# p2004dr/visual-slam

Hardware: AMD Instinct MI355X
Metric: frames/sec (extract+match+pose) at 640×480, 2000 ORB, 1/2/4/8 MI355X (higher is better)
Workload: dtype u8

## Files before the change

visual-slam_amd/csrc/orb_kernels.hip:

```cpp
#include <cstring>

#include "common.h"
#include "select_replay.h"

__constant__ __attribute__((aligned(16))) int8_t c_pattern[256 * 4] = {
#include "orb_pattern.inc"
};

#define WAVE 64

__device__ __forceinline__ int reflect101(int p, int len) {
    if (len == 1) return 0;
    while (p < 0 || p >= len) p = p < 0 ? -p : 2 * len - 2 - p;
    return p;
}

__device__ __forceinline__ void xcd_map(uint32_t lin, uint32_t per, uint32_t inv_per, uint32_t batch, int& frame, int& item) {
    const uint32_t b8 = batch & ~7u, cut = per * b8;
    const bool head = lin < cut;
    const uint32_t n = head ? lin >> 3 : lin - cut;
    const uint32_t q = inv_per ? __umulhi(n, inv_per) : n;
    item = (int)(n - q * per);
    frame = (int)(head ? (lin & 7u) + 8u * q : b8 + q);
}

__device__ __forceinline__ const uint8_t* level_ptr(const Plan& P, int L, const uint8_t* gray, const uint8_t* pyr,
                                                    int frame) {
    return L == 0 ? gray + (size_t)frame * P.w * P.h : pyr + (size_t)frame * P.pyr_stride + P.lv[L].off;
}

__global__ void k_gray(const uint8_t* __restrict__ bgr, uint8_t* __restrict__ gray, size_t npx) {
    size_t i = (size_t)blockIdx.x * blockDim.x + threadIdx.x;
    if (i >= npx) return;
    int b = bgr[3 * i], g = bgr[3 * i + 1], r = bgr[3 * i + 2];
    gray[i] = (uint8_t)((b * 3735 + g * 19235 + r * 9798 + (1 << 14)) >> 15);
}

int orb_launch_gray(mo_ctx* c, const uint8_t* d_bgr, int w, int h, int batch, uint8_t* d_gray) {
    size_t npx = (size_t)w * h * batch;
    hipLaunchKernelGGL(k_gray, dim3((unsigned)((npx + 255) / 256)), dim3(256), 0, c->stream, d_bgr, d_gray, npx);
    HIPCHK(c, hipGetLastError());
    return MO_OK;
}

__global__ __launch_bounds__(256) void k_ingest(const uint8_t* __restrict__ src, uint8_t* __restrict__ gray, int npx, int ch, int* flags_clear) {
    const int i = (blockIdx.x * 256 + threadIdx.x) * 16;
    if (blockIdx.x == 0 && threadIdx.x == 0 && flags_clear) { flags_clear[0] = 0; flags_clear[1] = 0; flags_clear[2] = 0; flags_clear[3] = 0; }
    if (i >= npx) return;
    if (i + 16 <= npx) {
        if (ch == 1) {
            *(uint4*)(gray + i) = *(const uint4*)(src + i);
        } else {
            const uint4* s4 = (const uint4*)(src + (size_t)3 * i);
            const uint4 a = s4[0], b = s4[1], c = s4[2];
            const uint32_t wsrc[12] = {a.x, a.y, a.z, a.w, b.x, b.y, b.z, b.w, c.x, c.y, c.z, c.w};
            uint32_t o[4];
#pragma unroll
            for (int q = 0; q < 4; q++) {
                uint32_t v = 0;
#pragma unroll
                for (int k = 0; k < 4; k++) {
                    const int byte = 3 * (4 * q + k);
                    const uint32_t bb = (wsrc[byte >> 2] >> (8 * (byte & 3))) & 255u, gg = (wsrc[(byte + 1) >> 2] >> (8 * ((byte + 1) & 3))) & 255u,
                                   rr = (wsrc[(byte + 2) >> 2] >> (8 * ((byte + 2) & 3))) & 255u;
                    v |= ((bb * 3735u + gg * 19235u + rr * 9798u + (1u << 14)) >> 15) << (8 * k);
                }
                o[q] = v;
            }
            *(uint4*)(gray + i) = make_uint4(o[0], o[1], o[2], o[3]);
        }
        return;
    }
    for (int j = i; j < npx; j++) {
        if (ch == 1) gray[j] = src[j];
        else gray[j] = (uint8_t)(((int)src[3 * (size_t)j] * 3735 + (int)src[3 * (size_t)j + 1] * 19235 + (int)src[3 * (size_t)j + 2] * 9798 + (1 << 14)) >> 15);
    }
}

int orb_launch_ingest(mo_ctx* c, const uint8_t* src_mapped, int w, int h, int ch, uint8_t* d_gray, int* flags_clear) {
    const int npx = w * h;
    hipLaunchKernelGGL(k_ingest, dim3((unsigned)((npx + 4095) / 4096)), dim3(256), 0, c->stream, src_mapped, d_gray, npx, ch, flags_clear);
    HIPCHK(c, hipGetLastError());
    return MO_OK;
}

typedef unsigned short u16x2 __attribute__((ext_vector_type(2)));
__device__ __forceinline__ uint32_t udot2(uint32_t a, uint32_t b, uint32_t c) {
    return __builtin_amdgcn_udot2(__builtin_bit_cast(u16x2, a), __builtin_bit_cast(u16x2, b), c, false);
}

#define RS_TW 64
#define RS_TH 64
#define RS_SRC_ROWS 136
#define RS_SRC_PITCH 144

__global__ __launch_bounds__(256) void k_resize(const uint8_t* __restrict__ src, size_t src_fstride, int spitch, int sw, int sh,
                                                uint8_t* __restrict__ dst, size_t dst_fstride, int dpitch, int dw, int dh,
                                                const int* __restrict__ xofs, const int* __restrict__ xc1,
                                                const int* __restrict__ yofs, const int* __restrict__ yc1,
                                                uint32_t inv_per, uint32_t inv_gx, int org) {
    __shared__ __attribute__((aligned(16))) uint8_t s_src[RS_SRC_ROWS * RS_SRC_PITCH];
    __shared__ int s_xo[RS_TW], s_xc[RS_TW], s_yo[RS_TH], s_yc[RS_TH];
    const int tid = threadIdx.x;
    int bx = blockIdx.x, by = blockIdx.y, bz = blockIdx.z;
    {
        int rem;
        xcd_map(bx + gridDim.x * (by + gridDim.y * bz), gridDim.x * gridDim.y, inv_per, gridDim.z, bz, rem);
        by = (int)(inv_gx ? __umulhi((uint32_t)rem, inv_gx) : (uint32_t)rem);
        bx = rem - by * (int)gridDim.x;
    }
    const int tx0 = org + bx * RS_TW, ty0 = org + by * RS_TH;
    const uint8_t* s = src + (size_t)bz * src_fstride;
    const int sx0 = xofs[tx0], sx1 = min(xofs[min(tx0 + RS_TW - 1, dw - 1)] + 1, sw - 1);
    const int sy0 = yofs[ty0], sy1 = min(yofs[min(ty0 + RS_TH - 1, dh - 1)] + 1, sh - 1);
    const int sxa = sx0 & ~3;
    const int ncols = sx1 - sxa + 1, nrows = sy1 - sy0 + 1;
    if (ncols > RS_SRC_PITCH || nrows > RS_SRC_ROWS) return;
    if (tid < RS_TW) {
        int x = min(tx0 + tid, dw - 1);
        s_xo[tid] = xofs[x];
        s_xc[tid] = xc1[x];
    } else if (tid < RS_TW + RS_TH) {
        int y = min(ty0 + tid - RS_TW, dh - 1);
        s_yo[tid - RS_TW] = yofs[y];
        s_yc[tid - RS_TW] = yc1[y];
    }
    if ((spitch & 3) == 0 && (((size_t)s) & 3) == 0) {
        const int ndw = (ncols + 3) >> 2;
        const uint32_t inv = 0x100000u / (uint32_t)ndw + 1u;
        const uint8_t* s0 = s + (size_t)sy0 * spitch + sxa;
        for (int i = tid; i < nrows * ndw; i += 256) {
            const uint32_t r = ((uint32_t)i * inv) >> 20, c4 = (uint32_t)i - r * (uint32_t)ndw;
            ((uint32_t*)(s_src + r * RS_SRC_PITCH))[c4] = *(const uint32_t*)(s0 + r * (uint32_t)spitch + 4u * c4);
        }
    } else {
        for (int i = tid; i < nrows * ncols; i += 256) {
            int r = i / ncols, cc = i - r * ncols;
            s_src[r * RS_SRC_PITCH + cc] = s[(size_t)(sy0 + r) * spitch + sxa + cc];
        }
    }
    __syncthreads();
    const int c0 = (tid & 15) * 4, x = tx0 + c0;
    if (x >= dw) return;
    int ox[4], ox1[4];
    uint32_t mx1[4];
#pragma unroll
    for (int k = 0; k < 4; k++) {
        ox[k] = s_xo[c0 + k] - sxa;
        ox1[k] = min(s_xo[c0 + k] + 1, sw - 1) - sxa;
        mx1[k] = s_xc[c0 + k];
    }
#pragma unroll
    for (int half = 0; half < RS_TH / 16; half++) {
        const int ry = (tid >> 4) + 16 * half, y = ty0 + ry;
        if (y >= dh) break;
        const int oy = s_yo[ry] - sy0, oy1 = min(s_yo[ry] + 1, sh - 1) - sy0;
        const uint32_t my1 = s_yc[ry], my0 = 256 - my1;
        const uint8_t* r0 = s_src + oy * RS_SRC_PITCH;
        const uint8_t* r1 = s_src + oy1 * RS_SRC_PITCH;
        uint32_t packed = 0;
#pragma unroll
        for (int k = 0; k < 4; k++) {
            const uint32_t mx0 = 256 - mx1[k];
            uint32_t h0 = mx0 * r0[ox[k]] + mx1[k] * r0[ox1[k]];
            uint32_t h1 = mx0 * r1[ox[k]] + mx1[k] * r1[ox1[k]];
            uint32_t v = my0 * h0 + my1 * h1;
            packed |= ((v + 32768u) >> 16) << (8 * k);
        }
        *(uint32_t*)(dst + (size_t)bz * dst_fstride + (size_t)y * dpitch + x) = packed;
    }
}


#define RS2_ROWS 136
#define RS2_UNR 5
__global__ __launch_bounds__(256) void k_resize2(const uint8_t* __restrict__ src, size_t src_fstride, int spitch, int sw, int sh,
                                                 uint8_t* __restrict__ dst, size_t dst_fstride, int dpitch, int dw, int dh,
                                                 const uint32_t* __restrict__ xpk, const uint32_t* __restrict__ ypk,
                                                 uint32_t inv_per, uint32_t inv_gx, int org) {
    __shared__ __attribute__((aligned(16))) uint2 s_h[RS2_ROWS][16];
    const int tid = threadIdx.x;
    int bx = blockIdx.x, by = blockIdx.y, bz = blockIdx.z;
    {
        int rem;
        xcd_map(bx + gridDim.x * (by + gridDim.y * bz), gridDim.x * gridDim.y, inv_per, gridDim.z, bz, rem);
        by = (int)(inv_gx ? __umulhi((uint32_t)rem, inv_gx) : (uint32_t)rem);
        bx = rem - by * (int)gridDim.x;
    }
    const int tx0 = org + bx * RS_TW, ty0 = org + by * RS_TH;
    const uint32_t ey0 = ypk[ty0], ey1 = ypk[min(ty0 + RS_TH - 1, dh - 1)];
    const int sy0 = (int)(ey0 & 0x7FFFu), sy1 = (int)(ey1 & 0x7FFFu) + (int)((ey1 >> 15) & 1u);
    const int nrows = sy1 - sy0 + 1;
    if (nrows > RS2_ROWS) return;
    const int cg = tid & 15, rr = tid >> 4;
    const uint4 xe = *(const uint4*)(xpk + tx0 + 4 * cg);
    uint32_t ye[RS_TH / 16];
#pragma unroll
    for (int half = 0; half < RS_TH / 16; half++) ye[half] = ypk[ty0 + rr + 16 * half];
    const uint32_t xk[4] = {xe.x, xe.y, xe.z, xe.w};
    const int ox0 = (int)(xk[0] & 0x7FFFu), ab = ox0 & ~3;
    const uint32_t sh8 = (uint32_t)(ox0 & 3);
    uint32_t sel[4], coef[4];
#pragma unroll
    for (int k = 0; k < 4; k++) {
        const uint32_t a = (xk[k] & 0x7FFFu) - (uint32_t)ox0, b = a + ((xk[k] >> 15) & 1u), c1 = xk[k] >> 16;
        sel[k] = a | (b << 16) | 0x0C000C00u;
        coef[k] = (256u - c1) | (c1 << 16);
    }
    const int o1 = min(ab + 4, spitch - 4), o2 = min(ab + 8, spitch - 4);
    const uint8_t* s0 = src + (size_t)bz * src_fstride + (size_t)sy0 * spitch;
    for (int r0 = rr; r0 < nrows; r0 += 16 * RS2_UNR) {
        uint32_t w[RS2_UNR][3];
#pragma unroll
        for (int i = 0; i < RS2_UNR; i++) {
            const uint8_t* row = s0 + (uint32_t)(min(r0 + 16 * i, nrows - 1) * spitch);
            w[i][0] = *(const uint32_t*)(row + ab); w[i][1] = *(const uint32_t*)(row + o1); w[i][2] = *(const uint32_t*)(row + o2);
        }
#pragma unroll
        for (int i = 0; i < RS2_UNR; i++) {
            const int r = r0 + 16 * i;
            if (r >= nrows) break;
            const uint32_t u0 = __builtin_amdgcn_alignbyte(w[i][1], w[i][0], sh8), u1 = __builtin_amdgcn_alignbyte(w[i][2], w[i][1], sh8);
            uint32_t hv[4];
#pragma unroll
            for (int k = 0; k < 4; k++) hv[k] = udot2(__builtin_amdgcn_perm(u1, u0, sel[k]), coef[k], 0u);
            s_h[r][cg] = make_uint2(hv[0] | (hv[1] << 16), hv[2] | (hv[3] << 16));
        }
    }
    __syncthreads();
    const int x = tx0 + 4 * cg;
    if (x >= dw) return;
#pragma unroll
    for (int half = 0; half < RS_TH / 16; half++) {
        const int y = ty0 + rr + 16 * half;
        if (y >= dh) break;
        const uint32_t e = ye[half], c1 = e >> 16, cy = (256u - c1) | (c1 << 16);
        const int oy = (int)(e & 0x7FFFu) - sy0, oy1 = oy + (int)((e >> 15) & 1u);
        const uint2 a = s_h[oy][cg], b = s_h[oy1][cg];
        const uint32_t v0 = udot2(__builtin_amdgcn_perm(b.x, a.x, 0x05040100u), cy, 32768u);
        const uint32_t v1 = udot2(__builtin_amdgcn_perm(b.x, a.x, 0x07060302u), cy, 32768u);
        const uint32_t v2 = udot2(__builtin_amdgcn_perm(b.y, a.y, 0x05040100u), cy, 32768u);
        const uint32_t v3 = udot2(__builtin_amdgcn_perm(b.y, a.y, 0x07060302u), cy, 32768u);
        const uint32_t packed = __builtin_amdgcn_perm(v1, v0, 0x0C0C0602u) | (__builtin_amdgcn_perm(v3, v2, 0x0C0C0602u) << 16);
        *(uint32_t*)(dst + (size_t)bz * dst_fstride + (size_t)y * dpitch + x) = packed;
    }
}

int orb_launch_pyramid(mo_ctx* c, const uint8_t* d_gray, int batch, int nlevels, int margin) {
    const Plan& P = c->plan;
    for (int L = 1; L < nlevels; L++) {
        const LevelInfo& s = P.lv[L - 1];
        const LevelInfo& d = P.lv[L];
        const uint8_t* src = L == 1 ? d_gray : c->d_pyr + s.off;
        size_t sfs = L == 1 ? (size_t)P.w * P.h : (size_t)P.pyr_stride;
        const ResizeTab& t = c->rtab[L];
        const int org = (d.w > 2 * margin + 8 && d.h > 2 * margin + 8) ? margin : 0;
        dim3 grid((d.w - 2 * org + RS_TW - 1) / RS_TW, (d.h - 2 * org + RS_TH - 1) / RS_TH, batch);
        const uint32_t per = grid.x * grid.y, inv_per = per > 1 ? 0xFFFFFFFFu / per + 1u : 0u, inv_gx = grid.x > 1 ? 0xFFFFFFFFu / grid.x + 1u : 0u;
        const bool al4 = ((((size_t)src) | sfs | (size_t)s.pitch) & 3) == 0 && s.pitch >= 12;
        if (al4 && t.two_pass_ok)
            hipLaunchKernelGGL(k_resize2, grid, dim3(256), 0, c->stream, src, sfs, s.pitch, s.w, s.h, c->d_pyr + d.off,
                               (size_t)P.pyr_stride, d.pitch, d.w, d.h, t.xpk, t.ypk, inv_per, inv_gx, org);
        else
            hipLaunchKernelGGL(k_resize, grid, dim3(256), 0, c->stream, src, sfs, s.pitch, s.w, s.h, c->d_pyr + d.off,
                               (size_t)P.pyr_stride, d.pitch, d.w, d.h, t.xofs, t.xc1, t.yofs, t.yc1, inv_per, inv_gx, org);
    }
    HIPCHK(c, hipGetLastError());
    return MO_OK;
}

#define BT_W 64
#define BT_QW (BT_W / 4)
#define BT_PP (256 / BT_QW)
#define BT_H 58
#define BT_PW (BT_W + 16)
#define BT_ROWS (BT_H + 6)


__device__ __forceinline__ uint32_t hi16_pair_sat_u8(uint32_t a, uint32_t b) {
    uint32_t d;
    asm("v_sat_pk_u8_i16 %0, %1" : "=v"(d) : "v"(__builtin_amdgcn_perm(b, a, 0x07060302u)));
    return d;
}

__global__ __launch_bounds__(256) void k_blur(Plan P, const uint32_t* __restrict__ tile_tab, uint32_t inv_per, int org,
                                              const uint8_t* __restrict__ gray, const uint8_t* __restrict__ pyr,
                                              uint8_t* __restrict__ blur) {
    __shared__ __attribute__((aligned(16))) uint8_t s_px[BT_ROWS * BT_PW];
    __shared__ __attribute__((aligned(16))) uint32_t s_row[(BT_ROWS / 2) * BT_W];
    int tile = blockIdx.x, frame = blockIdx.y;
    xcd_map(blockIdx.x + gridDim.x * blockIdx.y, gridDim.x, inv_per, gridDim.y, frame, tile);
    const uint32_t te = tile_tab[tile];
    const int L = te & 0xFF;
    const LevelInfo lv = P.lv[L];
    const int tx0 = org + (int)((te >> 8) & 0xFFF) * BT_W, ty0 = org + (int)(te >> 20) * BT_H;
    const uint8_t* img = level_ptr(P, L, gray, pyr, frame);
    const int tid = threadIdx.x;
    if ((lv.pitch & 3) == 0 && (((size_t)img) & 3) == 0) {
        auto stage = [&](int r, int c4) {
            const int y = reflect101(ty0 + r - 3, lv.h), x0 = tx0 - 4 + 4 * c4;
            const uint8_t* row = img + (uint32_t)(y * lv.pitch);
            uint32_t v;
            if (x0 >= 0 && x0 + 3 < lv.w) v = *(const uint32_t*)(row + x0);
            else {
                v = 0;
#pragma unroll
                for (int b = 0; b < 4; b++) v |= (uint32_t)row[reflect101(x0 + b, lv.w)] << (8 * b);
            }
            ((uint32_t*)(s_px + r * BT_PW))[c4] = v;
        };
        if (ty0 >= 3 && ty0 + BT_ROWS - 3 <= lv.h && tx0 >= 4 && tx0 + BT_W + 4 <= lv.w) {
            const uint8_t* base = img + (uint32_t)((ty0 - 3) * lv.pitch + tx0 - 4);
#pragma unroll
            for (int r = tid / BT_QW; r < BT_ROWS; r += BT_PP)
                ((uint32_t*)(s_px + r * BT_PW))[1 + tid % BT_QW] = *(const uint32_t*)(base + (uint32_t)(r * lv.pitch) + 4 + 4 * (tid % BT_QW));
            if (tid < 2 * BT_ROWS)
                ((uint32_t*)(s_px + (tid >> 1) * BT_PW))[(tid & 1) * (BT_QW + 1)] =
                    *(const uint32_t*)(base + (uint32_t)((tid >> 1) * lv.pitch) + (tid & 1) * (BT_W + 4));
        } else {
            for (int r = tid / BT_QW; r < BT_ROWS; r += BT_PP) stage(r, 1 + tid % BT_QW);
            for (int i = tid; i < 2 * BT_ROWS; i += 256) stage(i >> 1, (i & 1) * (BT_QW + 1));
        }
    } else {
        for (int i = tid; i < BT_ROWS * (BT_W + 6); i += 256) {
            int r = i / (BT_W + 6), cidx = i - r * (BT_W + 6);
            int y = reflect101(ty0 + r - 3, lv.h), x = reflect101(tx0 + cidx - 3, lv.w);
            s_px[r * BT_PW + cidx + 1] = img[(size_t)y * lv.pitch + x];
        }
    }
    __syncthreads();
    const uint32_t g0 = P.gk[0], g1 = P.gk[1], g2 = P.gk[2], g3 = P.gk[3];
#pragma unroll
    for (int h2 = 0; h2 < BT_ROWS / 2 / BT_PP; h2++) {
        const uint32_t ta = g0 | (g1 << 8) | (g2 << 16) | (g3 << 24), tb = g2 | (g1 << 8) | (g0 << 16);
        const int p = tid / BT_QW + BT_PP * h2, q = tid % BT_QW;
        uint32_t o[2][4];
#pragma unroll
        for (int h = 0; h < 2; h++) {
            const uint32_t* pw = (const uint32_t*)(s_px + (2 * p + h) * BT_PW + 4 * q);
            const uint32_t w0 = pw[0], w1 = pw[1], w2 = pw[2];
            o[h][0] = __builtin_amdgcn_udot4(__builtin_amdgcn_alignbyte(w1, w0, 1), ta, __builtin_amdgcn_udot4(__builtin_amdgcn_alignbyte(w2, w1, 1), tb, 0, false), false);
            o[h][1] = __builtin_amdgcn_udot4(__builtin_amdgcn_alignbyte(w1, w0, 2), ta, __builtin_amdgcn_udot4(__builtin_amdgcn_alignbyte(w2, w1, 2), tb, 0, false), false);
            o[h][2] = __builtin_amdgcn_udot4(__builtin_amdgcn_alignbyte(w1, w0, 3), ta, __builtin_amdgcn_udot4(__builtin_amdgcn_alignbyte(w2, w1, 3), tb, 0, false), false);
            o[h][3] = __builtin_amdgcn_udot4(w1, ta, __builtin_amdgcn_udot4(w2, tb, 0, false), false);
        }
        uint4 packed;
        packed.x = o[0][0] | (o[1][0] << 16);
        packed.y = o[0][1] | (o[1][1] << 16);
        packed.z = o[0][2] | (o[1][2] << 16);
        packed.w = o[0][3] | (o[1][3] << 16);
        *(uint4*)(&s_row[p * BT_W + 4 * q]) = packed;
    }
    __syncthreads();
#pragma unroll
    for (int h2 = 0; h2 < BT_ROWS / 2 / BT_PP; h2++) {
        const int p = tid / BT_QW + BT_PP * h2, c0 = (tid % BT_QW) * 4;
        const int x = tx0 + c0, y = ty0 + 2 * p;
        if (p < BT_H / 2 && y < lv.h && x < lv.w) {
            const uint32_t e0 = g0 | (g1 << 16), e1 = g2 | (g3 << 16), e2 = g2 | (g1 << 16), e3 = g0;
            const uint32_t d0 = g0 << 16, d1 = g1 | (g2 << 16), d2 = g3 | (g2 << 16), d3 = g1 | (g0 << 16);
            uint4 v[4];
#pragma unroll
            for (int j = 0; j < 4; j++) v[j] = *(const uint4*)(&s_row[(p + j) * BT_W + c0]);
            uint32_t se[4], so[4];
#pragma unroll
            for (int k = 0; k < 4; k++) {
                const uint32_t a0 = k == 0 ? v[0].x : k == 1 ? v[0].y : k == 2 ? v[0].z : v[0].w;
                const uint32_t a1 = k == 0 ? v[1].x : k == 1 ? v[1].y : k == 2 ? v[1].z : v[1].w;
                const uint32_t a2 = k == 0 ? v[2].x : k == 1 ? v[2].y : k == 2 ? v[2].z : v[2].w;
                const uint32_t a3 = k == 0 ? v[3].x : k == 1 ? v[3].y : k == 2 ? v[3].z : v[3].w;
                se[k] = udot2(a0, e0, udot2(a1, e1, udot2(a2, e2, udot2(a3, e3, 1u << 15))));
                so[k] = udot2(a0, d0, udot2(a1, d1, udot2(a2, d2, udot2(a3, d3, 1u << 15))));
            }
            const uint32_t pe = hi16_pair_sat_u8(se[0], se[1]) | (hi16_pair_sat_u8(se[2], se[3]) << 16);
            const uint32_t po = hi16_pair_sat_u8(so[0], so[1]) | (hi16_pair_sat_u8(so[2], so[3]) << 16);
            uint8_t* out = blur + (size_t)frame * P.blur_stride + lv.boff + (size_t)y * lv.bpitch + x;
            *(uint32_t*)out = pe;
            if (y + 1 < lv.h) *(uint32_t*)(out + lv.bpitch) = po;
        }
    }
}

int orb_launch_blur(mo_ctx* c, const uint8_t* d_gray, int batch, int nlevels, int margin) {
    const Plan& P = c->plan;
    if (nlevels < 1 || nlevels > P.nlevels) return mo_fail(c, MO_ERR_ARG, "blur: level count outside the plan");
    const int slot = margin > 0 ? 1 : 0;
    if (slot && c->tile_margin != margin && c->d_tile_tab[1]) { hipFree(c->d_tile_tab[1]); c->d_tile_tab[1] = nullptr; }
    if (!c->d_tile_tab[slot]) {
        std::vector<uint32_t> tab;
        for (int L = 0; L < P.nlevels; L++) {
            const int cw = std::max(P.lv[L].w - 2 * margin, 1), chh = std::max(P.lv[L].h - 2 * margin, 1);
            const int tx = (cw + BT_W - 1) / BT_W, ty = (chh + BT_H - 1) / BT_H;
            c->tile_cum[slot][L] = (int)tab.size();
            for (int y = 0; y < ty; y++)
                for (int x = 0; x < tx; x++) tab.push_back((uint32_t)L | ((uint32_t)x << 8) | ((uint32_t)y << 20));
        }
        c->tile_cum[slot][P.nlevels] = (int)tab.size();
        HIPCHK(c, hipMalloc((void**)&c->d_tile_tab[slot], tab.size() * sizeof(uint32_t)));
        HIPCHK(c, hipMemcpy(c->d_tile_tab[slot], tab.data(), tab.size() * sizeof(uint32_t), hipMemcpyHostToDevice));
        if (slot) c->tile_margin = margin;
    }
    const uint32_t per = (uint32_t)c->tile_cum[slot][nlevels], inv_per = per > 1 ? 0xFFFFFFFFu / per + 1u : 0u;
    hipLaunchKernelGGL(k_blur, dim3(per, batch), dim3(256), 0, c->stream, P, c->d_tile_tab[slot], inv_per, margin, d_gray, c->d_pyr,
                       c->d_blur);
    HIPCHK(c, hipGetLastError());
    return MO_OK;
}

__device__ __forceinline__ bool arc9(uint32_t m) {
    uint32_t m32 = m | (m << 16);
    uint32_t x = m32 & (m32 >> 1);
    x &= x >> 2;
    x &= x >> 4;
    x &= m32 >> 8;
    return (x & 0xFFFFu) != 0;
}

__device__ __forceinline__ int arc_score(const int d[16]) {
    int m2[16], m4[16], best = -1000;
#pragma unroll
    for (int i = 0; i < 16; i++) m2[i] = min(d[i], d[(i + 1) & 15]);
#pragma unroll
    for (int i = 0; i < 16; i++) m4[i] = min(m2[i], m2[(i + 2) & 15]);
#pragma unroll
    for (int i = 0; i < 16; i++) {
        int m8 = min(m4[i], m4[(i + 4) & 15]);
        int m9 = min(m8, d[(i + 8) & 15]);
        best = max(best, m9);
    }
    return best - 1;
}

#define FAST_LOAD_D(d, v, p, TW)                                                                              \
    d[0] = v - p[3 * TW];   d[1] = v - p[3 * TW + 1];   d[2] = v - p[2 * TW + 2];   d[3] = v - p[TW + 3];        \
    d[4] = v - p[3];        d[5] = v - p[-TW + 3];      d[6] = v - p[-2 * TW + 2];  d[7] = v - p[-3 * TW + 1];   \
    d[8] = v - p[-3 * TW];  d[9] = v - p[-3 * TW - 1];  d[10] = v - p[-2 * TW - 2]; d[11] = v - p[-TW - 3];      \
    d[12] = v - p[-3];      d[13] = v - p[TW - 3];      d[14] = v - p[2 * TW - 2];  d[15] = v - p[3 * TW - 1];

typedef short s16x2 __attribute__((ext_vector_type(2)));
__device__ __forceinline__ s16x2 pk_min(s16x2 a, s16x2 b) { return __builtin_elementwise_min(a, b); }
__device__ __forceinline__ s16x2 pk_max(s16x2 a, s16x2 b) { return __builtin_elementwise_max(a, b); }

__device__ __forceinline__ int sub16(int a, int b) { int r; asm("v_sub_u16 %0, %1, %2" : "=v"(r) : "v"(a), "v"(b)); return r; }
__device__ __forceinline__ int min16(int a, int b) { int r; asm("v_min_i16 %0, %1, %2" : "=v"(r) : "v"(a), "v"(b)); return r; }
__device__ __forceinline__ int max16(int a, int b) { int r; asm("v_max_i16 %0, %1, %2" : "=v"(r) : "v"(a), "v"(b)); return r; }
__device__ __forceinline__ unsigned long long ballot_gt16(int a, int b) {
    unsigned long long m;
    asm("v_cmp_gt_i16 %0, %1, %2" : "=s"(m) : "v"(a), "v"(b));
    return m;
}

__device__ __forceinline__ void lds_store_u16_masked(unsigned long long mask, uint32_t addr, uint32_t val) {
    unsigned long long keep;
    asm volatile("s_mov_b64 %0, exec\n\ts_and_b64 exec, exec, %1\n\tds_write_b16 %2, %3\n\ts_mov_b64 exec, %0"
                 : "=&s"(keep) : "s"(mask), "v"(addr), "v"(val) : "memory", "scc");
}

#define FAST_CORNER_CAP 896
#define FAST_KEEP_WORDS 512
#define FAST_STACK 384

template <int TW, int NT>
__global__ __launch_bounds__(NT) void k_fast(Plan P, const uint32_t* __restrict__ strip_tab, uint32_t inv_per, int strip0,
                                              const uint8_t* __restrict__ gray, const uint8_t* __restrict__ pyr,
                                              uint32_t* __restrict__ cand, int* __restrict__ strip_cnt, int score_bytes) {
    extern __shared__ __attribute__((aligned(16))) uint8_t smem[];
    int strip = blockIdx.x, frame = blockIdx.y;
    xcd_map(blockIdx.x + gridDim.x * blockIdx.y, gridDim.x, inv_per, gridDim.y, frame, strip);
    const uint32_t se = strip_tab[strip0 + strip];
    const int L = se & 0xFF;
    const LevelInfo lv = P.lv[L];
    strip = (int)(se >> 8);
    if (strip >= lv.nstrips) return;
    const int R = lv.strip_rows;
    const int y0 = lv.by0 + strip * R;
    const int rows = min(R, lv.by0 + lv.bh - y0);
    const int SW = lv.bw + 2;
    const int xs0 = lv.bx0 - 1;
    uint8_t* s_score = smem;
    uint8_t* s_tile = smem + score_bytes;
    constexpr int NW = NT / 64;
    __shared__ int s_wsum[NW];
    __shared__ __attribute__((aligned(16))) uint16_t s_wq[NW][FAST_STACK];
    __shared__ uint16_t s_corner[FAST_CORNER_CAP];
    __shared__ int s_ncorner;
    uint32_t* const s_keep = (uint32_t*)&s_wq[0][0];
    static_assert(sizeof(uint16_t) * NW * FAST_STACK >= 4 * FAST_KEEP_WORDS, "bitmap overlays the stacks");
    const uint8_t* img = level_ptr(P, L, gray, pyr, frame);
    const int t = P.fast_threshold;
    const int tid = threadIdx.x, lane = tid & 63;
    const int wv = __builtin_amdgcn_readfirstlane(tid >> 6);

    const bool al16 = (lv.pitch & 15) == 0 && (((size_t)img) & 15) == 0;
    const bool al4 = (lv.pitch & 3) == 0 && (((size_t)img) & 3) == 0;
    const int gx0 = al16 ? (xs0 - 3) & ~15 : (xs0 - 3) & ~3, lead = xs0 - 3 - gx0;
    const int th = rows + 8, gy0 = y0 - 4;
    if (al16) {
        const int tw16 = (SW + 6 + lead + 15) >> 4;
        const uint32_t inv = 0xFFFFFFFFu / (uint32_t)tw16 + 1u;
        for (int i = tid; i < th * tw16; i += NT) {
            const int r = tw16 > 1 ? (int)__umulhi((uint32_t)i, inv) : i, c16 = i - r * tw16;
            *(uint4*)(s_tile + r * TW + 16 * c16) = *(const uint4*)(img + (size_t)(gy0 + r) * lv.pitch + gx0 + 16 * c16);
        }
    } else if (al4) {
        const int tw4 = (SW + 6 + lead + 3) >> 2;
        for (int r = wv; r < th; r += NW) {
            const uint32_t* src = (const uint32_t*)(img + (size_t)(gy0 + r) * lv.pitch + gx0);
            uint32_t* dst = (uint32_t*)(s_tile + r * TW);
            for (int c4 = lane; c4 < tw4; c4 += 64) dst[c4] = src[c4];
        }
    } else {
        const int tw_used = (SW + 6 + lead + 3) & ~3;
        for (int r = wv; r < th; r += NW) {
            const uint8_t* src = img + (size_t)(gy0 + r) * lv.pitch + gx0;
            for (int cc = lane; cc < tw_used; cc += 64) s_tile[r * TW + cc] = (gx0 + cc < lv.w) ? src[cc] : 0;
        }
    }
    for (int i = tid; i < ((rows + 2) * SW + 3) >> 2; i += NT) ((uint32_t*)s_score)[i] = 0;
    if (tid == 0) s_ncorner = 0;
    __syncthreads();

    typedef const volatile __attribute__((address_space(3))) uint8_t lds_cvu8;
    const int t_list = max(t, 1);
    const int xbits = R > 8 ? 11 : 12;
    const uint32_t xmask = (1u << xbits) - 1u;
    auto score_one = [&](uint32_t e, int flip, bool own) {
        const int r = e >> xbits, x = e & xmask;
        const int pos = r * SW + x;
        lds_cvu8* p = (lds_cvu8*)&s_tile[(r + 3) * TW + x + 3 + lead];
        const int v = (int)p[0];
        int d[16];
#define FAST_D(k, o) d[k] = sub16(v, (int)p[o]);
        FAST_D(0, 3 * TW)        FAST_D(1, 3 * TW + 1)    FAST_D(2, 2 * TW + 2)    FAST_D(3, TW + 3)
        FAST_D(4, 3)             FAST_D(5, -TW + 3)       FAST_D(6, -2 * TW + 2)   FAST_D(7, -3 * TW + 1)
        FAST_D(8, -3 * TW)       FAST_D(9, -3 * TW - 1)   FAST_D(10, -2 * TW - 2)  FAST_D(11, -TW - 3)
        FAST_D(12, -3)           FAST_D(13, TW - 3)       FAST_D(14, 2 * TW - 2)   FAST_D(15, 3 * TW - 1)
#undef FAST_D
        auto lo = [flip](int a, int b2) { return flip ? max16(a, b2) : min16(a, b2); };
        auto hi = [flip](int a, int b2) { return flip ? min16(a, b2) : max16(a, b2); };
        int mn3[16];
#pragma unroll
        for (int i = 0; i < 16; i++) mn3[i] = lo(d[i], lo(d[(i + 1) & 15], d[(i + 2) & 15]));
        int Ls = lo(mn3[0], lo(mn3[3], mn3[6]));
#pragma unroll
        for (int i = 1; i < 16; i++) Ls = hi(Ls, lo(mn3[i], lo(mn3[(i + 3) & 15], mn3[(i + 6) & 15])));
        const int L = flip ? -(int)(short)Ls : (int)(short)Ls;
        const int b = (int)(short)L;
        if (own && b > t) s_score[pos] = (uint8_t)(b - 1);
        const bool c = own && b > t_list;
        const unsigned long long m = __ballot(c);
        if (m) {
            int base = 0;
            if (lane == 0) base = atomicAdd(&s_ncorner, __popcll(m));
            base = __builtin_amdgcn_readfirstlane(base);
            const int o = base + __builtin_amdgcn_mbcnt_hi((unsigned)(m >> 32), __builtin_amdgcn_mbcnt_lo((unsigned)m, 0u));
            if (c && o < FAST_CORNER_CAP) s_corner[o] = (uint16_t)pos;
        }
    };
    {
        uint16_t* wq = s_wq[wv];
        const int nxc = (SW + 63) >> 6;
        int qd = 0, qb = 0;
        int ra = 0, ja = wv, rb = 0, jb = wv + NW;
        while (ja >= nxc) { ja -= nxc; ra++; }
        while (jb >= nxc) { jb -= nxc; rb++; }
        const int tv = t, ntv = -t;
        auto chunk = [&](int r, int j) {
            const int x = (j << 6) + lane;
            const int rem = SW - (j << 6);
            const unsigned long long valid = rem >= 64 ? ~0ull : (1ull << rem) - 1ull;
            const uint8_t* w = &s_tile[r * TW + lead + min(x, SW - 1)];
            const int v = w[3 * TW + 3];
            const int d0 = sub16(v, w[6 * TW + 3]), d4 = sub16(v, w[3 * TW + 6]), d8 = sub16(v, w[3]), d12 = sub16(v, w[3 * TW]);
#ifdef FAST_COMPASS_ANY2
            const int mn_a = min16(d0, d4), mx_a = max16(d0, d4), mn_b = min16(d8, d12), mx_b = max16(d8, d12);
            const int second_hi = max16(max16(min16(mx_a, mx_b), mn_a), mn_b);
            const int second_lo = min16(min16(max16(mn_a, mn_b), mx_a), mx_b);
#else
            const int second_hi = max16(max16(min16(d0, d4), min16(d4, d8)), max16(min16(d8, d12), min16(d12, d0)));
            const int second_lo = min16(min16(max16(d0, d4), max16(d4, d8)), min16(max16(d8, d12), max16(d12, d0)));
#endif
            const unsigned long long md = ballot_gt16(second_hi, tv) & valid;
            const unsigned long long mb = ballot_gt16(ntv, second_lo) & valid;
            const uint32_t e = (uint32_t)((r << xbits) | x);
            const uint32_t wq_lds = (uint32_t)(uintptr_t)wq;
            lds_store_u16_masked(md, wq_lds + 2u * (uint32_t)(qd + __builtin_amdgcn_mbcnt_hi((unsigned)(md >> 32), __builtin_amdgcn_mbcnt_lo((unsigned)md, 0u))), e);
            qd += __popcll(md);
            lds_store_u16_masked(mb, wq_lds + 2u * (uint32_t)(FAST_STACK - 1 - qb - (int)__builtin_amdgcn_mbcnt_hi((unsigned)(mb >> 32), __builtin_amdgcn_mbcnt_lo((unsigned)mb, 0u))), e);
            qb += __popcll(mb);
        };
        while (ra < rows + 2) {
            chunk(ra, ja);
            if (rb < rows + 2) chunk(rb, jb);
            if (qd >= 64 || qb >= 64) {
                replay::wave_sync();
                while (qd >= 64) { qd -= 64; score_one(wq[qd + lane], 0, true); }
                while (qb >= 64) { qb -= 64; score_one(wq[FAST_STACK - 1 - qb - lane], 0xFF, true); }
                replay::wave_sync();
            }
            ja += 2 * NW;
            while (ja >= nxc) { ja -= nxc; ra++; }
            jb += 2 * NW;
            while (jb >= nxc) { jb -= nxc; rb++; }
        }
        replay::wave_sync();
        if (qd > 0) score_one(wq[min(lane, qd - 1)], 0, lane < qd);
        if (qb > 0) score_one(wq[FAST_STACK - 1 - min(lane, qb - 1)], 0xFF, lane < qb);
    }
    __syncthreads();
    for (int i = tid; i < FAST_KEEP_WORDS; i += NT) s_keep[i] = 0;
    __syncthreads();

    const int nitems = rows * lv.bw;
    {
        const int nc = s_ncorner;
        const uint32_t inv_sw = 0xFFFFFFFFu / (uint32_t)SW + 1u;
        auto nms_at = [&](int p) {
            const int r = (int)__umulhi((uint32_t)p, inv_sw), x = p - r * SW;
            if (r < 1 || r > rows || x < 1 || x > lv.bw) return;
            const uint8_t* c = &s_score[p];
            const int mid = c[0];
            const int nb = max(max(max((int)c[-SW - 1], (int)c[-SW]), max((int)c[-SW + 1], (int)c[-1])),
                               max(max((int)c[1], (int)c[SW - 1]), max((int)c[SW], (int)c[SW + 1])));
            if (mid > nb) {
                const int i = (r - 1) * lv.bw + (x - 1);
                atomicOr(&s_keep[i >> 5], 1u << (i & 31));
            }
        };
        if (nc <= FAST_CORNER_CAP) {
            for (int k = tid; k < nc; k += NT) nms_at(s_corner[k]);
        } else {
            const int nband = (rows + 2) * SW;
            for (int k = tid; 4 * k < nband; k += NT) {
                uint32_t w = ((const uint32_t*)s_score)[k];
#pragma unroll
                for (int bq = 0; bq < 4; bq++)
                    if (((w >> (8 * bq)) & 0xFFu) && 4 * k + bq < nband) nms_at(4 * k + bq);
            }
        }
    }
    __syncthreads();
    const int nwords = (nitems + 31) >> 5, wpt = (nwords + NT - 1) / NT;
    uint32_t kw[2] = {0u, 0u};
#pragma unroll
    for (int q = 0; q < 2; q++)
        if (q < wpt && tid * wpt + q < nwords) kw[q] = s_keep[tid * wpt + q];
    const int cnt = __popc(kw[0]) + __popc(kw[1]);
    int incl = cnt;
#pragma unroll
    for (int o = 1; o < 64; o <<= 1) {
        int n = __shfl_up(incl, o, 64);
        if (lane >= o) incl += n;
    }
    if (lane == 63) s_wsum[wv] = incl;
    __syncthreads();
    int base = 0;
    for (int k = 0; k < wv; k++) base += s_wsum[k];
    int total = 0;
    for (int k = 0; k < NW; k++) total += s_wsum[k];
    int pos = base + incl - cnt;
    uint32_t* out = cand + (size_t)frame * P.cand_stride + lv.cand_off + (size_t)strip * lv.strip_cap;
#pragma unroll
    for (int q = 0; q < 2; q++) {
        uint32_t bits = kw[q];
        while (bits) {
            const int j = __ffs((int)bits) - 1;
            bits &= bits - 1;
            const int i = (tid * wpt + q) * 32 + j;
            const int rr = lv.bw > 1 ? (int)__umulhi((uint32_t)i, lv.inv_bw) : i, xx = i - rr * lv.bw;
            const int sc = s_score[(rr + 1) * SW + xx + 1];
            if (pos < lv.strip_cap) out[pos] = ((uint32_t)sc << 24) | ((uint32_t)(y0 + rr) << 12) | (uint32_t)(lv.bx0 + xx);
            pos++;
        }
    }
    if (tid == 0) strip_cnt[(size_t)frame * P.strips_per_frame + lv.strip_base + strip] = min(total, lv.strip_cap);
}

template <int TW, int NT> static int launch_fast_tw(mo_ctx* c, const uint8_t* d_gray, int batch, size_t score_bytes, int max_rows,
                                                    int strip0, int nstrips) {
    const Plan& P = c->plan;
    size_t lds = score_bytes + (size_t)(max_rows + 8) * TW + 16;
    if (lds > 128 * 1024) return mo_fail(c, MO_ERR_UNSUPPORTED, "level too wide for the FAST strip kernel");
    const unsigned bit = (TW == 704 ? 1u : TW == 1344 ? 2u : TW == 2112 ? 4u : TW == 608 ? 32u : 8u) << (NT == 512 ? 8 : 0);
    if (!(c->lds_attr_done & bit)) {
        HIPCHK(c, hipFuncSetAttribute((const void*)k_fast<TW, NT>, hipFuncAttributeMaxDynamicSharedMemorySize, 128 * 1024));
        c->lds_attr_done |= bit;
    }
    if (!c->d_strip_tab) {
        std::vector<uint32_t> tab((size_t)P.strips_per_frame, 0xFFFFFF00u);
        for (int L = 0; L < P.nlevels; L++)
            for (int st = 0; st < P.lv[L].nstrips; st++) tab[(size_t)P.lv[L].strip_base + st] = (uint32_t)L | ((uint32_t)st << 8);
        HIPCHK(c, hipMalloc((void**)&c->d_strip_tab, tab.size() * sizeof(uint32_t)));
        HIPCHK(c, hipMemcpy(c->d_strip_tab, tab.data(), tab.size() * sizeof(uint32_t), hipMemcpyHostToDevice));
        c->n_strip_tab = (int)tab.size();
    }
    const uint32_t per = (uint32_t)nstrips, inv_per = per > 1 ? 0xFFFFFFFFu / per + 1u : 0u;
    hipLaunchKernelGGL((k_fast<TW, NT>), dim3(nstrips, batch), dim3(NT), lds, c->stream, P, c->d_strip_tab, inv_per, strip0, d_gray,
                       c->d_pyr, c->d_cand, c->d_strip_cnt, (int)score_bytes);
    HIPCHK(c, hipGetLastError());
    return MO_OK;
}

int orb_launch_fast(mo_ctx* c, const uint8_t* d_gray, int batch, int level_lo, int level_hi) {
    const Plan& P = c->plan;
    level_lo = std::max(level_lo, 0); level_hi = std::min(level_hi, P.nlevels);
    if (level_lo >= level_hi) return MO_OK;
    const int strip0 = P.lv[level_lo].strip_base;
    const int nstrips = (level_hi < P.nlevels ? P.lv[level_hi].strip_base : P.strips_per_frame) - strip0;
    if (nstrips < 1) return MO_OK;
    size_t score_bytes = 0;
    int tw_need = 0, max_rows = 1;
    for (int L = 0; L < P.nlevels; L++) {
        const LevelInfo& v = P.lv[L];
        score_bytes = std::max(score_bytes, (((size_t)(v.strip_rows + 2) * (v.bw + 2) + 15) & ~(size_t)15));
        tw_need = std::max(tw_need, (v.bw + 2 + 6 + 15 + 15) & ~15);
        max_rows = std::max(max_rows, v.strip_rows);
    }
    if (P.strips_per_frame < 1) return MO_OK;
    if (tw_need <= 608) return launch_fast_tw<608, 256>(c, d_gray, batch, score_bytes, max_rows, strip0, nstrips);
    if (tw_need <= 704) return launch_fast_tw<704, 256>(c, d_gray, batch, score_bytes, max_rows, strip0, nstrips);
    if (tw_need <= 1344) return launch_fast_tw<1344, 256>(c, d_gray, batch, score_bytes, max_rows, strip0, nstrips);
    if (tw_need <= 2112) return launch_fast_tw<2112, 256>(c, d_gray, batch, score_bytes, max_rows, strip0, nstrips);
    return launch_fast_tw<4160, 256>(c, d_gray, batch, score_bytes, max_rows, strip0, nstrips);
}

#ifndef SEL_BUF_KB
#define SEL_BUF_KB 46
#endif
#define SEL_BUF_BYTES (SEL_BUF_KB * 1024)

__device__ float harris_response(const uint8_t* img, int pitch, int x0, int y0) {
    int a = 0, b = 0, cc = 0;
    for (int i = -3; i <= 3; i++) {
        const uint8_t* pm = img + (size_t)(y0 + i - 1) * pitch + x0;
        const uint8_t* p0 = pm + pitch;
        const uint8_t* pp = p0 + pitch;
#pragma unroll
        for (int j = -3; j <= 3; j++) {
            int Ix = ((int)p0[j + 1] - (int)p0[j - 1]) * 2 + ((int)pm[j + 1] - (int)pm[j - 1]) +
                     ((int)pp[j + 1] - (int)pp[j - 1]);
            int Iy = ((int)pp[j] - (int)pm[j]) * 2 + ((int)pp[j - 1] - (int)pm[j - 1]) + ((int)pp[j + 1] - (int)pm[j + 1]);
            a += Ix * Ix;
            b += Iy * Iy;
            cc += Ix * Iy;
        }
    }
    const float scale = 1.f / ((1 << 2) * 7 * 255.f);
    const float scale_sq_sq = scale * scale * scale * scale;
    float fa = (float)a, fb = (float)b, fc = (float)cc;
    float t1 = fa * fb;
    float t2 = fc * fc;
    float s = fa + fb;
    float t3 = 0.04f * s;
    float t4 = t3 * s;
    return ((t1 - t2) - t4) * scale_sq_sq;
}

__device__ __forceinline__ size_t sel_need_bytes(int n, int rec_bytes) {
    return (((size_t)n * rec_bytes + 7) & ~(size_t)7) + ((((size_t)n / 2 + 1) * 2 + 7) & ~(size_t)7) + ((size_t)n / 64 + 8) * 8;
}

#define HG 8
#define SEL_THREADS 256
#define SEL_THREADS_LATENCY 1024

__device__ __forceinline__ void harris_fetch(const uint8_t* img, int pitch, int x0, int y0, int g, uint32_t (&reg)[4]) {
    const uint8_t* base = img + (size_t)(y0 - 4) * pitch + ((x0 - 4) & ~3);
#pragma unroll
    for (int k = 0; k < 4; k++) {
        const int q = min(g + HG * k, 26), r = q / 3, dw = q - 3 * r;
        reg[k] = *(const uint32_t*)(base + r * pitch + 4 * dw);
    }
}
__device__ __forceinline__ float harris_group(const uint32_t (&reg)[4], int x0, uint32_t* tile , int g) {
    const int off = (x0 - 4) & 3;
#pragma unroll
    for (int k = 0; k < 4; k++)
        if (g + HG * k < 27) tile[g + HG * k] = reg[k];
    replay::wave_sync();
    int a = 0, b = 0, c = 0;
    if (g < 7) {
        const uint8_t* col = (const uint8_t*)tile + off + 1 + g;
        int d[9], sm[9];
#pragma unroll
        for (int r = 0; r < 9; r++) {
            const int l = col[12 * r - 1], m = col[12 * r], rt = col[12 * r + 1];
            d[r] = rt - l;
            sm[r] = l + 2 * m + rt;
        }
#pragma unroll
        for (int r = 1; r < 8; r++) {
            const int Ix = d[r - 1] + 2 * d[r] + d[r + 1], Iy = sm[r + 1] - sm[r - 1];
            a += Ix * Ix; b += Iy * Iy; c += Ix * Iy;
        }
    }
#pragma unroll
    for (int o = 1; o < HG; o <<= 1) { a += __shfl_xor(a, o, 64); b += __shfl_xor(b, o, 64); c += __shfl_xor(c, o, 64); }
    replay::wave_sync();
    const float scale = 1.f / ((1 << 2) * 7 * 255.f);
    const float scale_sq_sq = scale * scale * scale * scale;
    float fa = (float)a, fb = (float)b, fc = (float)c;
    float t1 = fa * fb;
    float t2 = fc * fc;
    float sx = fa + fb;
    float t3 = 0.04f * sx;
    float t4 = t3 * sx;
    return ((t1 - t2) - t4) * scale_sq_sq;
}

template <int NT, class PA, class PB>
__device__ __forceinline__ void select_harris(const Plan& P, const LevelInfo& lv, const uint8_t* img, PA A, PB B, int N1,
                                              uint16_t* rpos, unsigned long long* bl, FinalKp* fin, int* fin_cnt_out,
                                              int* flags, replay::WgScratch<NT>* ws, uint32_t (*s_hw)[27] , int level) {
    const int tid = threadIdx.x;
    constexpr int HG_GROUPS = NT / HG;
    if ((lv.pitch & 3) == 0 && (((size_t)img) & 3) == 0) {
        const int grp = tid / HG, g = tid % HG;
#ifndef SEL_HB
#define SEL_HB 4
#endif
        constexpr int HB = SEL_HB;
        for (int i0 = 0; i0 < N1; i0 += HG_GROUPS * HB) {
            uint32_t e[HB], reg[HB][4];
#pragma unroll
            for (int u = 0; u < HB; u++) {
                e[u] = A[min(i0 + u * HG_GROUPS + grp, N1 - 1)];
                harris_fetch(img, lv.pitch, e[u] & 0xFFF, (e[u] >> 12) & 0xFFF, g, reg[u]);
            }
#pragma unroll
            for (int u = 0; u < HB; u++) {
                const int i = i0 + u * HG_GROUPS + grp;
                const float r = harris_group(reg[u], e[u] & 0xFFF, s_hw[grp], g);
                if (g == 0 && i < N1) B[i] = ((uint64_t)__float_as_uint(r) << 32) | (e[u] & 0xFFFFFFu);
            }
        }
    } else {
        for (int i = tid; i < N1; i += NT) {
            uint32_t e = A[i];
            int x = e & 0xFFF, y = (e >> 12) & 0xFFF;
            float r = harris_response(img, lv.pitch, x, y);
            B[i] = ((uint64_t)__float_as_uint(r) << 32) | (e & 0xFFFFFFu);
        }
    }
    __syncthreads();
    int N2 = replay::wg_retain_best<NT, uint64_t>(B, N1, lv.quota, P.select_order, rpos, bl, tid, ws);
    if (N2 > lv.fin_cap) {
        if (tid == 0) { atomicOr(&flags[0], 1); atomicOr(&flags[1], 1 << level); }
        N2 = lv.fin_cap;
    }
    for (int i = tid; i < N2; i += NT) {
        uint64_t e = B[i];
        FinalKp k;
        k.x = (uint16_t)(e & 0xFFF);
        k.y = (uint16_t)((e >> 12) & 0xFFF);
        k.response = __uint_as_float((uint32_t)(e >> 32));
        fin[i] = k;
    }
    if (tid == 0) *fin_cnt_out = N2;
}

template <int NT>
__global__ __launch_bounds__(NT) void k_select(Plan P, const uint8_t* __restrict__ gray, const uint8_t* __restrict__ pyr,
                                                        const uint32_t* __restrict__ cand, const int* __restrict__ strip_cnt,
                                                        uint64_t* __restrict__ scratch, size_t scratch_stride,
                                                        FinalKp* __restrict__ fin_all, int* __restrict__ fin_cnt, int* flags,
                                                        int level0, int buf_bytes, int* __restrict__ desc_todo) {
    extern __shared__ __attribute__((aligned(16))) uint8_t s_buf[];
    int* const s_pref = (int*)(s_buf + buf_bytes);
    __shared__ replay::WgScratch<NT> s_ws;
    __shared__ uint32_t s_hw[NT / HG][27];
    const int L = level0 + blockIdx.y, frame = blockIdx.x, tid = threadIdx.x;
    if (desc_todo && frame == 0 && blockIdx.y == 0 && tid == 0) desc_todo[0] = 0;
    const LevelInfo lv = P.lv[L];
    int* fin_cnt_out = &fin_cnt[(size_t)frame * MO_MAX_LEVELS + L];
    if (lv.nstrips == 0) {
        if (tid == 0) *fin_cnt_out = 0;
        return;
    }
    const int* cnts = strip_cnt + (size_t)frame * P.strips_per_frame + lv.strip_base;
    for (int s = tid; s < lv.nstrips; s += NT) s_pref[s + 1] = cnts[s];
    __syncthreads();
    if (tid == 0) {
        s_pref[0] = 0;
        for (int s = 0; s < lv.nstrips; s++) s_pref[s + 1] += s_pref[s];
    }
    __syncthreads();
    const int N = s_pref[lv.nstrips];
    uint64_t* scr = scratch + (size_t)frame * scratch_stride + lv.scr_off;
    uint64_t* gB = scr;
    uint32_t* gA = (uint32_t*)(scr + lv.cand_cap);
    uint16_t* g_rpos = (uint16_t*)(gA + lv.cand_cap + (lv.cand_cap & 1));
    unsigned long long* g_bl = (unsigned long long*)(g_rpos + (((size_t)lv.cand_cap / 2 + 4) & ~(size_t)3));
    const bool a_lds = sel_need_bytes(N, 4) <= (size_t)buf_bytes;
    uint32_t* s_A = (uint32_t*)s_buf;
    uint16_t* a_rpos = (uint16_t*)(s_buf + (((size_t)N * 4 + 7) & ~(size_t)7));
    unsigned long long* a_bl = (unsigned long long*)((uint8_t*)a_rpos + ((((size_t)N / 2 + 1) * 2 + 7) & ~(size_t)7));
    const uint32_t* src = cand + (size_t)frame * P.cand_stride + lv.cand_off;
    {
        const int lane = tid & 63, wv = tid >> 6;
        constexpr int NW = NT / 64, GU = 4;
        for (int s0 = wv; s0 < lv.nstrips; s0 += NW * GU) {
            uint32_t v[GU];
            int b[GU], n[GU];
#pragma unroll
            for (int u = 0; u < GU; u++) {
                const int st = min(s0 + u * NW, lv.nstrips - 1);
                b[u] = s_pref[st];
                n[u] = s0 + u * NW < lv.nstrips ? s_pref[st + 1] - b[u] : 0;
                v[u] = lane < n[u] ? src[(size_t)st * lv.strip_cap + lane] : 0u;
            }
#pragma unroll
            for (int u = 0; u < GU; u++) {
                if (lane < n[u]) { if (a_lds) s_A[b[u] + lane] = v[u]; else gA[b[u] + lane] = v[u]; }
                if (n[u] > WAVE) {
                    const uint32_t* e = src + (size_t)(s0 + u * NW) * lv.strip_cap;
                    for (int i = WAVE + lane; i < n[u]; i += WAVE) { if (a_lds) s_A[b[u] + i] = e[i]; else gA[b[u] + i] = e[i]; }
                }
            }
        }
    }
    __syncthreads();
    const int N1 = a_lds ? replay::wg_retain_best<NT, uint32_t>(s_A, N, 2 * lv.quota, P.select_order, a_rpos, a_bl, tid, &s_ws)
                         : replay::wg_retain_best<NT, uint32_t>(gA, N, 2 * lv.quota, P.select_order, g_rpos, g_bl, tid, &s_ws);
    const size_t b_off = a_lds ? (((size_t)N1 * 4 + 15) & ~(size_t)15) : 0;
    const bool b_lds = b_off + sel_need_bytes(N1, 8) <= (size_t)buf_bytes;
    uint64_t* s_B = (uint64_t*)(s_buf + b_off);
    uint16_t* b_rpos = (uint16_t*)((uint8_t*)s_B + (size_t)N1 * 8);
    unsigned long long* b_bl = (unsigned long long*)((uint8_t*)b_rpos + ((((size_t)N1 / 2 + 1) * 2 + 7) & ~(size_t)7));
    const uint8_t* img = level_ptr(P, L, gray, pyr, frame);
    FinalKp* fin = fin_all + (size_t)frame * P.fin_stride + lv.fin_off;
    if (a_lds && b_lds) select_harris<NT>(P, lv, img, s_A, s_B, N1, b_rpos, b_bl, fin, fin_cnt_out, flags, &s_ws, s_hw, L);
    else if (a_lds) select_harris<NT>(P, lv, img, s_A, gB, N1, g_rpos, g_bl, fin, fin_cnt_out, flags, &s_ws, s_hw, L);
    else if (b_lds) select_harris<NT>(P, lv, img, gA, s_B, N1, b_rpos, b_bl, fin, fin_cnt_out, flags, &s_ws, s_hw, L);
    else select_harris<NT>(P, lv, img, gA, gB, N1, g_rpos, g_bl, fin, fin_cnt_out, flags, &s_ws, s_hw, L);
}

int orb_launch_select(mo_ctx* c, const uint8_t* d_gray, int batch, int level_lo, int level_hi) {
    const Plan& P = c->plan;
    level_lo = std::max(level_lo, 0); level_hi = std::min(level_hi, P.nlevels);
    if (level_lo >= level_hi) return MO_OK;
    for (int L = 0; L < P.nlevels; L++)
        if (P.lv[L].nstrips > SEL_MAXSTRIPS) return mo_fail(c, MO_ERR_UNSUPPORTED, "too many strips per level");
// ... 566 lines not shown
```

Baseline: 108,300.

## Score FAST on raw pixels with arc-extreme network and per-wave NMS queues

FAST scoring now works on raw pixel values. A shared prefix/suffix min-max network (fast_arc_extreme) computes the 9-arc extreme once and subtracts the center afterwards, replacing the 16 per-pixel differences and the redundant min3 chains. The compass pre-test compares v±t against pairwise extremes of the four cardinal pixels using unsigned 16-bit ops. The global atomic corner list with its overflow fallback is removed; NMS instead scans the score band per wave, compacting nonzero positions into per-wave LDS queues and processing them 64 at a time. This trades an extra full scan of the score buffer for fewer ALU ops and no block-level atomics.

```diff
diff --git a/visual-slam_amd/csrc/fast_score.h b/visual-slam_amd/csrc/fast_score.h
--- /dev/null
+++ b/visual-slam_amd/csrc/fast_score.h
@@ -0,0 +1,32 @@
+#pragma once
+
+#if defined(__HIPCC__) || defined(__HIP__)
+#define FAST_HD __host__ __device__ __forceinline__
+#else
+#define FAST_HD inline
+#endif
+
+template <class In, class Out>
+FAST_HD int fast_arc_extreme(const int p[16], In in, Out out) {
+    int s0[9];
+    s0[8] = p[8];
+#pragma unroll
+    for (int i = 7; i >= 0; i--) s0[i] = in(p[i], s0[i + 1]);
+    int a1[9], b1[9];
+    a1[0] = p[9];
+#pragma unroll
+    for (int j = 1; j < 9; j++) a1[j] = in(a1[j - 1], p[(9 + j) & 15]);
+    b1[8] = p[1];
+#pragma unroll
+    for (int i = 7; i >= 1; i--) b1[i] = in(p[(9 + i) & 15], b1[i + 1]);
+    int a2[6];
+    a2[0] = p[2];
+#pragma unroll
+    for (int j = 1; j < 6; j++) a2[j] = in(a2[j - 1], p[2 + j]);
+    int r = out(s0[0], a1[8]);
+#pragma unroll
+    for (int i = 1; i < 9; i++) r = out(r, in(s0[i], a1[i - 1]));
+#pragma unroll
+    for (int i = 10; i < 16; i++) r = out(r, in(b1[i - 9], a2[i - 10]));
+    return r;
+}
diff --git a/visual-slam_amd/csrc/orb_kernels.hip b/visual-slam_amd/csrc/orb_kernels.hip
--- a/visual-slam_amd/csrc/orb_kernels.hip
+++ b/visual-slam_amd/csrc/orb_kernels.hip
@@ -2,6 +2,7 @@
 
 #include "common.h"
 #include "select_replay.h"
+#include "fast_score.h"
 
 __constant__ __attribute__((aligned(16))) int8_t c_pattern[256 * 4] = {
 #include "orb_pattern.inc"
@@ -444,6 +445,9 @@
 __device__ __forceinline__ int sub16(int a, int b) { int r; asm("v_sub_u16 %0, %1, %2" : "=v"(r) : "v"(a), "v"(b)); return r; }
 __device__ __forceinline__ int min16(int a, int b) { int r; asm("v_min_i16 %0, %1, %2" : "=v"(r) : "v"(a), "v"(b)); return r; }
 __device__ __forceinline__ int max16(int a, int b) { int r; asm("v_max_i16 %0, %1, %2" : "=v"(r) : "v"(a), "v"(b)); return r; }
+__device__ __forceinline__ int add16(int a, int b) { int r; asm("v_add_u16 %0, %1, %2" : "=v"(r) : "v"(a), "v"(b)); return r; }
+__device__ __forceinline__ int min16u(int a, int b) { int r; asm("v_min_u16 %0, %1, %2" : "=v"(r) : "v"(a), "v"(b)); return r; }
+__device__ __forceinline__ int max16u(int a, int b) { int r; asm("v_max_u16 %0, %1, %2" : "=v"(r) : "v"(a), "v"(b)); return r; }
 __device__ __forceinline__ unsigned long long ballot_gt16(int a, int b) {
     unsigned long long m;
     asm("v_cmp_gt_i16 %0, %1, %2" : "=s"(m) : "v"(a), "v"(b));
@@ -456,9 +460,9 @@
                  : "=&s"(keep) : "s"(mask), "v"(addr), "v"(val) : "memory", "scc");
 }
 
-#define FAST_CORNER_CAP 896
 #define FAST_KEEP_WORDS 512
 #define FAST_STACK 384
+#define FAST_NMS_Q 128
 
 template <int TW, int NT>
 __global__ __launch_bounds__(NT) void k_fast(Plan P, const uint32_t* __restrict__ strip_tab, uint32_t inv_per, int strip0,
@@ -482,10 +486,8 @@
     constexpr int NW = NT / 64;
     __shared__ int s_wsum[NW];
     __shared__ __attribute__((aligned(16))) uint16_t s_wq[NW][FAST_STACK];
-    __shared__ uint16_t s_corner[FAST_CORNER_CAP];
-    __shared__ int s_ncorner;
     uint32_t* const s_keep = (uint32_t*)&s_wq[0][0];
-    static_assert(sizeof(uint16_t) * NW * FAST_STACK >= 4 * FAST_KEEP_WORDS, "bitmap overlays the stacks");
+    static_assert(sizeof(uint16_t) * NW * FAST_STACK >= 4 * FAST_KEEP_WORDS + sizeof(uint16_t) * NW * FAST_NMS_Q, "bitmap and queues overlay the stacks");
     const uint8_t* img = level_ptr(P, L, gray, pyr, frame);
     const int t = P.fast_threshold;
     const int tid = threadIdx.x, lane = tid & 63;
@@ -517,11 +519,9 @@
         }
     }
     for (int i = tid; i < ((rows + 2) * SW + 3) >> 2; i += NT) ((uint32_t*)s_score)[i] = 0;
-    if (tid == 0) s_ncorner = 0;
     __syncthreads();
 
     typedef const volatile __attribute__((address_space(3))) uint8_t lds_cvu8;
-    const int t_list = max(t, 1);
     const int xbits = R > 8 ? 11 : 12;
     const uint32_t xmask = (1u << xbits) - 1u;
     auto score_one = [&](uint32_t e, int flip, bool own) {
@@ -529,33 +529,18 @@
         const int pos = r * SW + x;
         lds_cvu8* p = (lds_cvu8*)&s_tile[(r + 3) * TW + x + 3 + lead];
         const int v = (int)p[0];
-        int d[16];
-#define FAST_D(k, o) d[k] = sub16(v, (int)p[o]);
-        FAST_D(0, 3 * TW)        FAST_D(1, 3 * TW + 1)    FAST_D(2, 2 * TW + 2)    FAST_D(3, TW + 3)
-        FAST_D(4, 3)             FAST_D(5, -TW + 3)       FAST_D(6, -2 * TW + 2)   FAST_D(7, -3 * TW + 1)
-        FAST_D(8, -3 * TW)       FAST_D(9, -3 * TW - 1)   FAST_D(10, -2 * TW - 2)  FAST_D(11, -TW - 3)
-        FAST_D(12, -3)           FAST_D(13, TW - 3)       FAST_D(14, 2 * TW - 2)   FAST_D(15, 3 * TW - 1)
-#undef FAST_D
-        auto lo = [flip](int a, int b2) { return flip ? max16(a, b2) : min16(a, b2); };
-        auto hi = [flip](int a, int b2) { return flip ? min16(a, b2) : max16(a, b2); };
-        int mn3[16];
-#pragma unroll
-        for (int i = 0; i < 16; i++) mn3[i] = lo(d[i], lo(d[(i + 1) & 15], d[(i + 2) & 15]));
-        int Ls = lo(mn3[0], lo(mn3[3], mn3[6]));
-#pragma unroll
-        for (int i = 1; i < 16; i++) Ls = hi(Ls, lo(mn3[i], lo(mn3[(i + 3) & 15], mn3[(i + 6) & 15])));
-        const int L = flip ? -(int)(short)Ls : (int)(short)Ls;
+        int q[16];
+#define FAST_P(k, o) q[k] = (int)p[o];
+        FAST_P(0, 3 * TW)        FAST_P(1, 3 * TW + 1)    FAST_P(2, 2 * TW + 2)    FAST_P(3, TW + 3)
+        FAST_P(4, 3)             FAST_P(5, -TW + 3)       FAST_P(6, -2 * TW + 2)   FAST_P(7, -3 * TW + 1)
+        FAST_P(8, -3 * TW)       FAST_P(9, -3 * TW - 1)   FAST_P(10, -2 * TW - 2)  FAST_P(11, -TW - 3)
+        FAST_P(12, -3)           FAST_P(13, TW - 3)       FAST_P(14, 2 * TW - 2)   FAST_P(15, 3 * TW - 1)
+#undef FAST_P
+        auto mn = [](int a, int b2) { return min16u(a, b2); };
+        auto mx = [](int a, int b2) { return max16u(a, b2); };
+        const int L = flip ? sub16(fast_arc_extreme(q, mn, mx), v) : sub16(v, fast_arc_extreme(q, mx, mn));
         const int b = (int)(short)L;
         if (own && b > t) s_score[pos] = (uint8_t)(b - 1);
-        const bool c = own && b > t_list;
-        const unsigned long long m = __ballot(c);
-        if (m) {
-            int base = 0;
-            if (lane == 0) base = atomicAdd(&s_ncorner, __popcll(m));
-            base = __builtin_amdgcn_readfirstlane(base);
-            const int o = base + __builtin_amdgcn_mbcnt_hi((unsigned)(m >> 32), __builtin_amdgcn_mbcnt_lo((unsigned)m, 0u));
-            if (c && o < FAST_CORNER_CAP) s_corner[o] = (uint16_t)pos;
-        }
     };
     {
         uint16_t* wq = s_wq[wv];
@@ -564,24 +549,18 @@
         int ra = 0, ja = wv, rb = 0, jb = wv + NW;
         while (ja >= nxc) { ja -= nxc; ra++; }
         while (jb >= nxc) { jb -= nxc; rb++; }
-        const int tv = t, ntv = -t;
+        const int tv = t;
         auto chunk = [&](int r, int j) {
             const int x = (j << 6) + lane;
             const int rem = SW - (j << 6);
             const unsigned long long valid = rem >= 64 ? ~0ull : (1ull << rem) - 1ull;
             const uint8_t* w = &s_tile[r * TW + lead + min(x, SW - 1)];
             const int v = w[3 * TW + 3];
-            const int d0 = sub16(v, w[6 * TW + 3]), d4 = sub16(v, w[3 * TW + 6]), d8 = sub16(v, w[3]), d12 = sub16(v, w[3 * TW]);
-#ifdef FAST_COMPASS_ANY2
-            const int mn_a = min16(d0, d4), mx_a = max16(d0, d4), mn_b = min16(d8, d12), mx_b = max16(d8, d12);
-            const int second_hi = max16(max16(min16(mx_a, mx_b), mn_a), mn_b);
-            const int second_lo = min16(min16(max16(mn_a, mn_b), mx_a), mx_b);
-#else
-            const int second_hi = max16(max16(min16(d0, d4), min16(d4, d8)), max16(min16(d8, d12), min16(d12, d0)));
-            const int second_lo = min16(min16(max16(d0, d4), max16(d4, d8)), min16(max16(d8, d12), max16(d12, d0)));
-#endif
-            const unsigned long long md = ballot_gt16(second_hi, tv) & valid;
-            const unsigned long long mb = ballot_gt16(ntv, second_lo) & valid;
+            const int p0 = w[6 * TW + 3], p4 = w[3 * TW + 6], p8 = w[3], p12 = w[3 * TW];
+            const int pair_hi = min16u(min16u(max16u(p0, p4), max16u(p4, p8)), min16u(max16u(p8, p12), max16u(p12, p0)));
+            const int pair_lo = max16u(max16u(min16u(p0, p4), min16u(p4, p8)), max16u(min16u(p8, p12), min16u(p12, p0)));
+            const unsigned long long md = ballot_gt16(sub16(v, tv), pair_hi) & valid;
+            const unsigned long long mb = ballot_gt16(pair_lo, add16(v, tv)) & valid;
             const uint32_t e = (uint32_t)((r << xbits) | x);
             const uint32_t wq_lds = (uint32_t)(uintptr_t)wq;
             lds_store_u16_masked(md, wq_lds + 2u * (uint32_t)(qd + __builtin_amdgcn_mbcnt_hi((unsigned)(md >> 32), __builtin_amdgcn_mbcnt_lo((unsigned)md, 0u))), e);
@@ -613,31 +592,42 @@
 
     const int nitems = rows * lv.bw;
     {
-        const int nc = s_ncorner;
         const uint32_t inv_sw = 0xFFFFFFFFu / (uint32_t)SW + 1u;
         auto nms_at = [&](int p) {
             const int r = (int)__umulhi((uint32_t)p, inv_sw), x = p - r * SW;
             if (r < 1 || r > rows || x < 1 || x > lv.bw) return;
             const uint8_t* c = &s_score[p];
             const int mid = c[0];
-            const int nb = max(max(max((int)c[-SW - 1], (int)c[-SW]), max((int)c[-SW + 1], (int)c[-1])),
-                               max(max((int)c[1], (int)c[SW - 1]), max((int)c[SW], (int)c[SW + 1])));
-            if (mid > nb) {
+            const int nb = max16u(max16u(max16u((int)c[-SW - 1], (int)c[-SW]), max16u((int)c[-SW + 1], (int)c[-1])),
+                                  max16u(max16u((int)c[1], (int)c[SW - 1]), max16u((int)c[SW], (int)c[SW + 1])));
+            if ((uint16_t)mid > (uint16_t)nb) {
                 const int i = (r - 1) * lv.bw + (x - 1);
                 atomicOr(&s_keep[i >> 5], 1u << (i & 31));
             }
         };
-        if (nc <= FAST_CORNER_CAP) {
-            for (int k = tid; k < nc; k += NT) nms_at(s_corner[k]);
-        } else {
-            const int nband = (rows + 2) * SW;
-            for (int k = tid; 4 * k < nband; k += NT) {
-                uint32_t w = ((const uint32_t*)s_score)[k];
-#pragma unroll
-                for (int bq = 0; bq < 4; bq++)
-                    if (((w >> (8 * bq)) & 0xFFu) && 4 * k + bq < nband) nms_at(4 * k + bq);
-            }
-        }
+        uint16_t* const nq = (uint16_t*)(s_keep + FAST_KEEP_WORDS) + wv * FAST_NMS_Q;
+        const uint32_t nq_lds = (uint32_t)(uintptr_t)nq;
+        const int k_end = ((rows + 1) * SW + 3) >> 2;
+        int qn = 0;
+        for (int k0 = (SW >> 2) + (wv << 6); k0 < k_end; k0 += NT) {
+            const int k = k0 + lane;
+            const uint32_t w = k < k_end ? ((const uint32_t*)s_score)[k] : 0u;
+#pragma unroll
+            for (int bq = 0; bq < 4; bq++) {
+                const unsigned long long m = __ballot((w & (0xFFu << (8 * bq))) != 0u);
+                lds_store_u16_masked(m, nq_lds + 2u * (uint32_t)(qn + __builtin_amdgcn_mbcnt_hi((unsigned)(m >> 32), __builtin_amdgcn_mbcnt_lo((unsigned)m, 0u))),
+                                     (uint32_t)(4 * k + bq));
+                qn += __popcll(m);
+                if (qn >= 64) {
+                    replay::wave_sync();
+                    qn -= 64;
+                    nms_at(nq[qn + lane]);
+                    replay::wave_sync();
+                }
+            }
+        }
+        replay::wave_sync();
+        if (lane < qn) nms_at(nq[lane]);
     }
     __syncthreads();
     const int nwords = (nitems + 31) >> 5, wpt = (nwords + NT - 1) / NT;
```

New measurement: 116,300, median of 6. 7.4% higher.
